# enordber/pepr

Measured on AMD Instinct MI355X. Metric: M site-lnL/sec (WAG+G4 full-tree likelihood evaluations x alignment patterns); the gene-trees/sec half of BASELINE.json's metric is search.gene_trees_per_sec, higher is better.
Workload: dtype f64

## Files before the change

### pepr_amd/csrc/kernels.hip

```cpp
#include "kernels.h"
#include <hip/hip_ext.h>

#include <algorithm>
#include <cstdlib>

namespace pml {

#define TWO_P256 1.15792089237316195423570985008687907853269984665640564039457584007913129639936e77
#define TWO_M256 8.63616855509444462538635186280017219262570580443837358382049248904e-78
#define LOG_2_256 177.445678223345993274051579105116

__device__ __forceinline__ double mfma4(double a, double b, double c) {
#ifdef ABL_NO_MFMA
    return __builtin_fma(a, b, c);
#endif
    return __builtin_amdgcn_mfma_f64_4x4x4f64(a, b, c, 0, 0, 0);
}

__device__ __forceinline__ unsigned code_mask(unsigned code) {
    return code < 20u ? (1u << code) : (code == 20u ? 0xCu : (code == 21u ? 0x60u : 0xFFFFFu));
}

template <int CTRL>
__device__ __forceinline__ double quad_swap(double v) {
// ... 334 lines not shown
typedef double dvec2 __attribute__((ext_vector_type(2)));
typedef int ivec2 __attribute__((ext_vector_type(2)));
typedef unsigned uvec4 __attribute__((ext_vector_type(4)));
struct Operand {
    dvec2 v[5];
};

typedef const __attribute__((address_space(1))) char *gcptr;
typedef __attribute__((address_space(1))) char *gptr;
#define GLOBAL_AS __attribute__((address_space(1)))

__device__ __forceinline__ void load_clv(Operand &o, gcptr base, unsigned lane_off, size_t rowbytes, int c) {
#ifdef ABL_NO_CLV
    { for (int kk = 0; kk < 5; ++kk) o.v[kk] = (dvec2){0.05 + 1e-12 * lane_off, 0.05}; return; }
#endif
#pragma unroll
    for (int kk = 0; kk < 5; ++kk)
        o.v[kk] = __builtin_nontemporal_load(reinterpret_cast<const GLOBAL_AS dvec2 *>(base + (size_t)(c * NS + kk * 4) * rowbytes + lane_off));
}
__device__ __forceinline__ void load_tip(Operand &o, const unsigned char *__restrict__ T, unsigned codes, int q) {
    const unsigned char *t0 = T + (codes & 0xFFu) * NS + q, *t1 = T + (codes >> 8) * NS + q;
#pragma unroll
    for (int kk = 0; kk < 5; ++kk) o.v[kk] = (dvec2){(double)t0[kk * 4], (double)t1[kk * 4]};
}

__device__ __forceinline__ void contract(double (&acc)[5][2], const double *__restrict__ frag_c, const Operand &o) {
#ifdef ABL_NO_LDS
#define FRAG_RD(x) (0.05 + 1.0e-4 * (double)(&(x) - frag_c))
#else
#define FRAG_RD(x) (x)
#endif
    double a[2][5];
#pragma unroll
    for (int st = 0; st < 5; ++st) { acc[st][0] = 0.0; acc[st][1] = 0.0; a[0][st] = FRAG_RD(frag_c[(st * 5) * 16]); }
#pragma unroll
    for (int kk = 0; kk < 5; ++kk) {
        if (kk + 1 < 5) {
#pragma unroll
            for (int st = 0; st < 5; ++st) a[(kk + 1) & 1][st] = FRAG_RD(frag_c[(st * 5 + kk + 1) * 16]);
        }
#pragma unroll
        for (int st = 0; st < 5; ++st) {
            acc[st][0] = mfma4(a[kk & 1][st], o.v[kk].x, acc[st][0]);
            acc[st][1] = mfma4(a[kk & 1][st], o.v[kk].y, acc[st][1]);
        }
        __builtin_amdgcn_sched_barrier(0);
    }
}

template <typename F>
__device__ __forceinline__ void contract_stream(const double *__restrict__ frag_c, const Operand &o, F &&consume) {
    double a[2][5];
#pragma unroll
    for (int kk = 0; kk < 5; ++kk) a[0][kk] = FRAG_RD(frag_c[kk * 16]);
#pragma unroll
    for (int st = 0; st < 5; ++st) {
        if (st + 1 < 5) {
#pragma unroll
            for (int kk = 0; kk < 5; ++kk) a[(st + 1) & 1][kk] = FRAG_RD(frag_c[((st + 1) * 5 + kk) * 16]);
        }
        double acc0 = 0.0, acc1 = 0.0;
#pragma unroll
        for (int kk = 0; kk < 5; ++kk) {
            acc0 = mfma4(a[st & 1][kk], o.v[kk].x, acc0);
            acc1 = mfma4(a[st & 1][kk], o.v[kk].y, acc1);
        }
        consume(st, acc0, acc1);
        __builtin_amdgcn_sched_barrier(0);
    }
}

struct Rows5 { dvec2 a, b; double c; };
__device__ __forceinline__ Rows5 load_rows(const double *tab, unsigned code, int c, int q) {
#ifdef ABL_NO_ROWS
    { Rows5 r1; r1.a = (dvec2){0.9, 0.9}; r1.b = (dvec2){0.9, 0.9}; r1.c = 0.9 + 1e-9 * code; return r1; }
#endif
    gcptr p = (gcptr)tab + (size_t)((c * NCODES + code) * 4 + q) * (TIPTAB_KK * 8);
    Rows5 r;
    r.a = *reinterpret_cast<const GLOBAL_AS dvec2 *>(p);
    r.b = *reinterpret_cast<const GLOBAL_AS dvec2 *>(p + 16);
    r.c = *reinterpret_cast<const GLOBAL_AS double *>(p + 32);
    return r;
}
__device__ __forceinline__ void load_cherry(Operand &o, const OpSide &sd, unsigned ca, unsigned cb, int c, int q) {
    const Rows5 a0 = load_rows(sd.t0, ca & 0xFFu, c, q), a1 = load_rows(sd.t0, ca >> 8, c, q);
    const Rows5 b0 = load_rows(sd.t1, cb & 0xFFu, c, q), b1 = load_rows(sd.t1, cb >> 8, c, q);
    o.v[0] = (dvec2){a0.a.x * b0.a.x, a1.a.x * b1.a.x};
    o.v[1] = (dvec2){a0.a.y * b0.a.y, a1.a.y * b1.a.y};
    o.v[2] = (dvec2){a0.b.x * b0.b.x, a1.b.x * b1.b.x};
    o.v[3] = (dvec2){a0.b.y * b0.b.y, a1.b.y * b1.b.y};
    o.v[4] = (dvec2){a0.c * b0.c, a1.c * b1.c};
}
template <bool EARLY = true>
__device__ __forceinline__ void load_pitch(Operand &o, const OpSide &sd, const double *__restrict__ f_inner,
                                           unsigned ca, unsigned cb, unsigned cc, int c, int q) {
    Operand w;
    load_cherry(w, sd, ca, cb, c, q);
    Rows5 r0, r1;
    if (EARLY) { r0 = load_rows(sd.t2, cc & 0xFFu, c, q); r1 = load_rows(sd.t2, cc >> 8, c, q); }
    double v[5][2];
    contract(v, f_inner + c * 25 * 16, w);
    if (!EARLY) { r0 = load_rows(sd.t2, cc & 0xFFu, c, q); r1 = load_rows(sd.t2, cc >> 8, c, q); }
    o.v[0] = (dvec2){v[0][0] * r0.a.x, v[0][1] * r1.a.x};
    o.v[1] = (dvec2){v[1][0] * r0.a.y, v[1][1] * r1.a.y};
    o.v[2] = (dvec2){v[2][0] * r0.b.x, v[2][1] * r1.b.x};
    o.v[3] = (dvec2){v[3][0] * r0.b.y, v[3][1] * r1.b.y};
    o.v[4] = (dvec2){v[4][0] * r0.c, v[4][1] * r1.c};
}

template <bool CHAIN, bool FUSE>
__device__ __forceinline__ void chunk_op(const NvOp &op, const double *__restrict__ sP, const unsigned char *__restrict__ sT,
                                         int p, int lane, Operand (&X)[4], ivec2 &xsc) {
    const int q = lane >> 4;
    constexpr size_t rowbytes = (size_t)TILE_PAT * 8;
    const size_t tabrow = (size_t)op.mpad * 8;
    const unsigned lane_off = (unsigned)(p >> 7) * (unsigned)(CLV_ROWS * rowbytes) + (unsigned)((size_t)q * rowbytes) + (unsigned)(p & (TILE_PAT - 1)) * 8u;
    const int lk = op.flags & 3, rk = (op.flags >> 2) & 3;
    const bool nt_store = (op.flags & OPF_NT_STORE) != 0;
    const int mode = op.mode;
    const bool chL = CHAIN && (op.flags & OPF_CHAIN_L) != 0, chR = CHAIN && (op.flags & OPF_CHAIN_R) != 0;
    const bool fusedN = FUSE && (op.flags & OPF_FUSED_NEWTON) != 0;
    const bool keep = !(CHAIN && (op.flags & OPF_NO_STORE) != 0) && !fusedN;
    OpSide sdl = op.l, sdr = op.r;
    const int *l_scl = op.l_scl, *r_scl = op.r_scl; int *out_scl = op.out_scl; double *outp = op.out;
#define PML_PIN(x) asm volatile("" : "+s"(x))
    PML_PIN(sdl.p0); PML_PIN(sdl.p1); PML_PIN(sdl.p2); PML_PIN(sdl.t0); PML_PIN(sdl.t1); PML_PIN(sdl.t2); PML_PIN(sdl.f);
    PML_PIN(sdr.p0); PML_PIN(sdr.p1); PML_PIN(sdr.p2); PML_PIN(sdr.t0); PML_PIN(sdr.t1); PML_PIN(sdr.t2); PML_PIN(sdr.f);
    PML_PIN(l_scl); PML_PIN(r_scl); PML_PIN(out_scl); PML_PIN(outp);
    gcptr Lp = (gcptr)sdl.p0, Rp = (gcptr)sdr.p0;
    gptr O = (gptr)outp;
    const __amdgpu_buffer_rsrc_t orsrc = __builtin_amdgcn_make_buffer_rsrc((void *)outp, 0, 0x7FFFFFFF, 0x00020000);
    const double *fL = sP + (q * 4 + (lane & 3));
    const double *fR = fL + PFRAG;
    unsigned mx0 = 0u, mx1 = 0u;
    double site0 = 0.0, site1 = 0.0;
    unsigned cl = 0, cl2 = 0, cl3 = 0, cr = 0, cr2 = 0, cr3 = 0;
    const double *fLi = fL + 2 * PFRAG;
    const bool both_pitch = lk == SK_PITCH && rk == SK_PITCH;
    const double *fRg = sdr.f + (q * 4 + (lane & 3));
#ifdef ABL_NO_CODES
#define CODE_LD(ptr) ((((unsigned)p * 5u + 1u + (unsigned)(size_t)(ptr)) % 20u) | ((((unsigned)p * 3u + 2u) % 20u) << 8))
#else
#define CODE_LD(ptr) (*reinterpret_cast<const GLOBAL_AS unsigned short *>(ptr))
#endif
    if (lk != SK_CLV) cl = CODE_LD(Lp + p);
    if (lk >= SK_CHERRY) cl2 = CODE_LD((gcptr)sdl.p1 + p);
    if (lk == SK_PITCH) cl3 = CODE_LD((gcptr)sdl.p2 + p);
    if (rk != SK_CLV) cr = CODE_LD(Rp + p);
    if (rk >= SK_CHERRY) cr2 = CODE_LD((gcptr)sdr.p1 + p);
    if (rk == SK_PITCH) cr3 = CODE_LD((gcptr)sdr.p2 + p);

    const bool lookL = mode < MODE_EVALUATE && lk == SK_TIP && !__any((cl & 0xFFu) >= 20u || (cl >> 8) >= 20u);
    const bool lookR = mode < MODE_EVALUATE && rk == SK_TIP && !__any((cr & 0xFFu) >= 20u || (cr >> 8) >= 20u);
    const double *tL0 = sP + ((cl & 0xFFu) >> 2) * 16 + (cl & 3u) * 4 + q, *tL1 = sP + ((cl >> 8) >> 2) * 16 + ((cl >> 8) & 3u) * 4 + q;
    const double *tR0 = sP + PFRAG + ((cr & 0xFFu) >> 2) * 16 + (cr & 3u) * 4 + q, *tR1 = sP + PFRAG + ((cr >> 8) >> 2) * 16 + ((cr >> 8) & 3u) * 4 + q;
    Operand curL, curR;
    if (lk == SK_TIP && !lookL) load_tip(curL, sT, cl, q);
    else if (lk == SK_CLV && !chL) load_clv(curL, Lp, lane_off, rowbytes, 0);
    if (rk == SK_TIP && !lookR) load_tip(curR, sT, cr, q);
    else if (rk == SK_CLV && !chR) load_clv(curR, Rp, lane_off, rowbytes, 0);
    constexpr bool DIRECT_IN = CHAIN && !FUSE;
    constexpr int CAT_UNROLL = CHAIN ? NCAT : 1;
#pragma unroll CAT_UNROLL
    for (int c = 0; c < NCAT; ++c) {
        if (FUSE) { if (chL) curL = X[c]; if (chR) curR = X[c]; }
        if (lk == SK_CHERRY) load_cherry(curL, sdl, cl, cl2, c, q);
        else if (lk == SK_PITCH) load_pitch<!FUSE>(curL, sdl, fLi, cl, cl2, cl3, c, q);
        if (rk == SK_CHERRY) load_cherry(curR, sdr, cr, cr2, c, q);
        else if (rk == SK_PITCH) { if (both_pitch) load_pitch<!FUSE>(curR, sdr, fRg, cr, cr2, cr3, c, q); else load_pitch<!FUSE>(curR, sdr, fLi, cr, cr2, cr3, c, q); }
        if (mode >= MODE_EVALUATE) {
            if (DIRECT_IN && chL) contract_stream(fR + c * 25 * 16, curR, [&](int st, double y0, double y1) { site0 += X[c].v[st].x * y0; site1 += X[c].v[st].y * y1; });
            else if (DIRECT_IN && chR) contract_stream(fR + c * 25 * 16, X[c], [&](int st, double y0, double y1) { site0 += curL.v[st].x * y0; site1 += curL.v[st].y * y1; });
            else contract_stream(fR + c * 25 * 16, curR, [&](int st, double y0, double y1) {
                site0 += curL.v[st].x * y0; site1 += curL.v[st].y * y1;
            });
            if (mode == MODE_EVALUATE_CAT) {
                double a0 = site0, a1 = site1;
                a0 += __shfl_xor(a0, 16); a0 += __shfl_xor(a0, 32);
                a1 += __shfl_xor(a1, 16); a1 += __shfl_xor(a1, 32);
                if (q == 0) *reinterpret_cast<GLOBAL_AS dvec2 *>(O + (size_t)c * tabrow + 8 * p) = (dvec2){a0, a1};
                site0 = 0.0; site1 = 0.0;
            }
        } else {
            double aL[5][2];
            if (lookL) {
#pragma unroll
                for (int st = 0; st < 5; ++st) { aL[st][0] = tL0[c * 400 + st * 80]; aL[st][1] = tL1[c * 400 + st * 80]; }
            } else if (DIRECT_IN && chL) contract(aL, fL + c * 25 * 16, X[c]);
            else contract(aL, fL + c * 25 * 16, curL);
            auto emit = [&](int st, double y0, double y1) {
                const double o0 = aL[st][0] * y0, o1 = aL[st][1] * y1;
                mx0 = max(mx0, (unsigned)__double2hiint(o0)); mx1 = max(mx1, (unsigned)__double2hiint(o1));
                if (CHAIN) X[c].v[st] = (dvec2){o0, o1};
                if (!keep) return;
#ifdef ABL_NO_STORE
                return;
#endif
                const uvec4 bits = __builtin_bit_cast(uvec4, ((dvec2){o0, o1}));
                const int soff = (c * NS + st * 4) * (int)rowbytes;
                if (nt_store) __builtin_amdgcn_raw_buffer_store_b128(bits, orsrc, lane_off, soff, 2);
                else __builtin_amdgcn_raw_buffer_store_b128(bits, orsrc, lane_off, soff, 0);
            };
            if (lookR) {
#pragma unroll
                for (int st = 0; st < 5; ++st) emit(st, tR0[c * 400 + st * 80], tR1[c * 400 + st * 80]);
            } else contract_stream(fR + c * 25 * 16, curR, emit);
        }
        if (c + 1 < NCAT) {
            if (lk == SK_CLV && !chL) load_clv(curL, Lp, lane_off, rowbytes, c + 1);
            if (rk == SK_CLV && !chR) load_clv(curR, Rp, lane_off, rowbytes, c + 1);
        }
    }

    ivec2 sc = {0, 0};
    if (q == 0) {
        if (lk == SK_CLV) { if (chL) sc += xsc; else sc += *reinterpret_cast<const GLOBAL_AS ivec2 *>((gcptr)l_scl + 4 * p); }
        if (rk == SK_CLV) { if (chR) sc += xsc; else sc += *reinterpret_cast<const GLOBAL_AS ivec2 *>((gcptr)r_scl + 4 * p); }
    }
    if (mode == MODE_NEWVIEW) {
        mx0 = max(mx0, (unsigned)__shfl_xor((int)mx0, 16)); mx0 = max(mx0, (unsigned)__shfl_xor((int)mx0, 32));
        mx1 = max(mx1, (unsigned)__shfl_xor((int)mx1, 16)); mx1 = max(mx1, (unsigned)__shfl_xor((int)mx1, 32));
        constexpr unsigned HI_TWO_M256 = (1023u - 256u) << 20;
        const bool n0 = mx0 < HI_TWO_M256, n1 = mx1 < HI_TWO_M256;
        if (__any(n0 || n1)) {
            if (CHAIN) {
                const double f0 = n0 ? TWO_P256 : 1.0, f1 = n1 ? TWO_P256 : 1.0;
#pragma unroll
                for (int c = 0; c < NCAT; ++c)
#pragma unroll
                    for (int k = 0; k < 5; ++k) { X[c].v[k].x *= f0; X[c].v[k].y *= f1; }
            }
            if (keep && (n0 || n1)) {
#pragma unroll 1
                for (int r = 0; r < NCAT * 5; ++r) {
                    GLOBAL_AS dvec2 *ptr = reinterpret_cast<GLOBAL_AS dvec2 *>(O + (size_t)((r / 5) * NS + (r % 5) * 4) * rowbytes + lane_off);
                    dvec2 v = *ptr;
                    if (n0) v.x *= TWO_P256;
                    if (n1) v.y *= TWO_P256;
                    *ptr = v;
                }
            }
        }
        if (q == 0) { sc.x += n0 ? 1 : 0; sc.y += n1 ? 1 : 0; if (keep) *reinterpret_cast<GLOBAL_AS ivec2 *>((gptr)out_scl + 4 * p) = sc; }
        if (CHAIN) xsc = sc;
    } else if (mode == MODE_SUMTABLE || mode == MODE_EVALUATE_CAT) {
        if (fusedN) xsc = sc;
        else if (q == 0) *reinterpret_cast<GLOBAL_AS ivec2 *>((gptr)out_scl + 4 * p) = sc;
    } else {
        site0 += __shfl_xor(site0, 16); site0 += __shfl_xor(site0, 32);
        site1 += __shfl_xor(site1, 16); site1 += __shfl_xor(site1, 32);
        if (q == 0) {
            const double l0 = log(site0 * 0.25) - sc.x * LOG_2_256;
            const double l1 = log(site1 * 0.25) - sc.y * LOG_2_256;
            *reinterpret_cast<GLOBAL_AS dvec2 *>(O + 8 * p) = (dvec2){l0, l1};
        }
    }
}

constexpr int PAT_PER_WG = 4 * PAT_PER_WAVE;
constexpr int TIPTAB = NCODES * NS;

#ifndef PML_CHAIN_WAVES
#define PML_CHAIN_WAVES 2
#endif
__device__ __forceinline__ void dma_chunk(const double *set, double *lds_set, int k, int lane) {
    const GLOBAL_AS char *src = (const GLOBAL_AS char *)set + k * 4096 + lane * 16;
    __attribute__((address_space(3))) char *dst = (__attribute__((address_space(3))) char *)lds_set + k * 4096;
    if (k < 3) {
        __builtin_amdgcn_global_load_lds((const GLOBAL_AS void *)src, (__attribute__((address_space(3))) void *)dst, 16, 0, 0);
        __builtin_amdgcn_global_load_lds((const GLOBAL_AS void *)src, (__attribute__((address_space(3))) void *)dst, 16, 1024, 0);
        __builtin_amdgcn_global_load_lds((const GLOBAL_AS void *)src, (__attribute__((address_space(3))) void *)dst, 16, 2048, 0);
        __builtin_amdgcn_global_load_lds((const GLOBAL_AS void *)src, (__attribute__((address_space(3))) void *)dst, 16, 3072, 0);
    } else if (lane < 32) __builtin_amdgcn_global_load_lds((const GLOBAL_AS void *)src, (__attribute__((address_space(3))) void *)dst, 16, 0, 0);
}
__device__ __forceinline__ void stage_frags_dma3(const NvOp &op, double *dst, int lane, int wave) {
    const int wv = __builtin_amdgcn_readfirstlane(wave);
    const double *pl = op.pl, *pr = op.pr;
    const int lk = op.flags & 3, rk = (op.flags >> 2) & 3;
    const double *inner = (lk == SK_PITCH) ? op.l.f : (rk == SK_PITCH) ? op.r.f : nullptr;
    dma_chunk(pl ? pl : pr, dst, wv, lane);
    dma_chunk(pr ? pr : pl, dst + PFRAG, (wv + 1) & 3, lane);
    if (inner != nullptr) dma_chunk(inner, dst + 2 * PFRAG, (wv + 2) & 3, lane);
}

struct FusedShared {
    double exl[NCAT * NS][2];
    double red[3];
    double fb[3][PAT_PER_WAVE * 4];
    double ss[PAT_PER_WAVE * 4];
    double bc[4];
};
static_assert(sizeof(FusedShared) <= PFRAG * sizeof(double), "fused Newton scratch fits one fragment region");
__device__ __forceinline__ void newton_fused(const NvOp &op, double *scratch, const Operand (&X)[4], const ivec2 xsc,
                                             bool active, int blk, NewtonCtl *ctl, long long timeout_ticks) {
    const NewtonReq &r = *reinterpret_cast<const NewtonReq *>(op.aux);
    FusedShared &sh = *reinterpret_cast<FusedShared *>(scratch);
    const int tid = threadIdx.x, lane = tid & 63, wave = tid >> 6, q = lane >> 4, pl = wave * PAT_PER_WAVE + 2 * (lane & 15);
    const int mpad = r.mpad, S = newton_split(mpad);
    const ModelDev *__restrict__ md = r.md;
    u64 *gran = reinterpret_cast<u64 *>(r.sync);
    __syncthreads();
    if (q == 0) { sh.ss[pl] = active ? (double)xsc.x : 0.0; sh.ss[pl + 1] = active ? (double)xsc.y : 0.0; }
    if (tid == 0) sh.bc[3] = 0.0;
    double sw = 0.0;
    if (wave < 2) { const int pf = blk * (PAT_PER_WAVE * 4) + wave * 64 + lane; if (pf < mpad) sw = r.weight[pf]; }
    int nevals = 0;
    auto eval_at = [&](double t, double &L, double &d1, double &d2) -> bool {
        if (tid < NCAT * NS) {
            const double lr = md->eval[tid % NS] * r.rates[tid / NS];
            sh.exl[tid][0] = exp(lr * t); sh.exl[tid][1] = lr;
        }
        __syncthreads();
        double fa = 0.0, fa1 = 0.0, fa2 = 0.0, fb = 0.0, fb1 = 0.0, fb2 = 0.0;
#pragma unroll
        for (int c = 0; c < NCAT; ++c)
#pragma unroll
            for (int st = 0; st < 5; ++st) {
                const int row = c * NS + 4 * st + q;
                const double e = sh.exl[row][0], lr = sh.exl[row][1];
                newton_term(X[c].v[st].x, e, lr, fa, fa1, fa2);
                newton_term(X[c].v[st].y, e, lr, fb, fb1, fb2);
            }
        fa += __shfl_xor(fa, 16); fa += __shfl_xor(fa, 32); fa1 += __shfl_xor(fa1, 16); fa1 += __shfl_xor(fa1, 32); fa2 += __shfl_xor(fa2, 16); fa2 += __shfl_xor(fa2, 32);
        fb += __shfl_xor(fb, 16); fb += __shfl_xor(fb, 32); fb1 += __shfl_xor(fb1, 16); fb1 += __shfl_xor(fb1, 32); fb2 += __shfl_xor(fb2, 16); fb2 += __shfl_xor(fb2, 32);
        if (q == 0) {
            sh.fb[0][pl] = fa; sh.fb[1][pl] = fa1; sh.fb[2][pl] = fa2;
            sh.fb[0][pl + 1] = fb; sh.fb[1][pl + 1] = fb1; sh.fb[2][pl + 1] = fb2;
        }
        __syncthreads();
        double tot[3] = {0.0, 0.0, 0.0};
        if (wave < 2) {
            double a0 = 0.0, a1 = 0.0, a2 = 0.0;
            if (sw != 0.0) {
                const int j = wave * 64 + lane;
                newton_finish(sh.fb[0][j], sh.fb[1][j], sh.fb[2][j], sw, sh.ss[j], a0, a1, a2);
            }
            tot[0] = wave_sum(a0); tot[1] = wave_sum(a1); tot[2] = wave_sum(a2);
            if (wave == 0 && lane == 0) { sh.red[0] = tot[0]; sh.red[1] = tot[1]; sh.red[2] = tot[2]; }
        }
        __syncthreads();
        if (wave == 1) {
#pragma unroll
            for (int i = 0; i < 3; ++i) tot[i] = sh.red[i] + __shfl(tot[i], 0);
            bool bad = false;
            if (S > 1) bad = newton_exchange(gran, S, blk, nevals, r.tag_base, tot, ctl, timeout_ticks);
            if (lane == 0) { sh.bc[0] = tot[0]; sh.bc[1] = tot[1]; sh.bc[2] = tot[2]; if (bad) sh.bc[3] = 1.0; }
        }
        __syncthreads();
        ++nevals;
        L = uni(sh.bc[0]); d1 = uni(sh.bc[1]); d2 = uni(sh.bc[2]);
        return sh.bc[3] == 0.0;
    };
    double t, L, d1, d2;
    const bool ok = newton_drive(r.t0, r.max_iter, r.tol, eval_at, t, L, d1, d2);
    if (tid == 64 && blk == 0) {
        atomicAdd(&ctl->n_requests, 1ull); atomicAdd(&ctl->n_evals, (unsigned long long)nevals);
        if (!ok) { t = r.t0; L = __builtin_nan(""); }
        r.out[0] = t; r.out[1] = L; r.out[2] = d1; r.out[3] = d2;
        if (r.t_dev0) { *r.t_dev0 = t; *r.t_dev1 = t; }
    }
}

#ifdef PML_OPTIME
__device__ unsigned long long g_optime[256][2];
}
extern "C" void pml_abl_optime(unsigned long long *out, int reset) {
    (void)hipDeviceSynchronize();
    (void)hipMemcpyFromSymbol(out, HIP_SYMBOL(pml::g_optime), sizeof(unsigned long long) * 512);
    if (reset) { static unsigned long long z[512]; (void)hipMemcpyToSymbol(HIP_SYMBOL(pml::g_optime), z, sizeof z); }
}
namespace pml {
#endif
template <bool CHAIN, bool DBUF, bool FUSE>
__global__ __launch_bounds__(256, CHAIN ? PML_CHAIN_WAVES : 4) void k_oplist(
        const NvOp *__restrict__ ops, const GeneRun *__restrict__ runs, int nruns, int blocks_per_gene, int any_pitch,
        NewtonCtl *ctl, long long timeout_ticks) {
    static_assert(CHAIN || !DBUF, "LDS-DMA staging exists for the chained kernels only");
    static_assert(!FUSE || (CHAIN && DBUF), "the fused-Newton kernel is the scoring kernel plus the Newton code");
#ifdef PML_OPTIME
    const long long t_life0 = clock64();
#endif
    constexpr int PARITY_STRIDE = 3 * PFRAG;
    Operand X[4]; ivec2 xsc = {0, 0};
#pragma unroll
    for (int c = 0; c < 4; ++c)
#pragma unroll
        for (int k = 0; k < 5; ++k) X[c].v[k] = (dvec2){0.0, 0.0};
    extern __shared__ double sP[];
    const int nfrag_regions = DBUF ? 6 : 2 + (any_pitch ? 1 : 0);
    unsigned char *sT = reinterpret_cast<unsigned char *>(sP + nfrag_regions * PFRAG);
    const int tid = threadIdx.x, lane = tid & 63, wave = tid >> 6;
    const bool one_part = blocks_per_gene < 0;
    if (one_part) blocks_per_gene = -blocks_per_gene;
    const int xcd = one_part ? 0 : (blockIdx.x & 7);
    int slot = one_part ? (int)blockIdx.x : (int)(blockIdx.x >> 3);
    const bool ticketed = FUSE && ctl != nullptr;
    if (ticketed) {
        __shared__ int s_slot;
        if (tid == 0) s_slot = __hip_atomic_fetch_add(&ctl->oticket[xcd], 1, __ATOMIC_RELAXED, __HIP_MEMORY_SCOPE_AGENT);
        __syncthreads();
        slot = s_slot;
    }
    auto leave = [&]() {
        if (!ticketed) return;
        __syncthreads();
        if (tid == 0) {
            const int d = __hip_atomic_fetch_add(&ctl->odone, 1, __ATOMIC_RELAXED, __HIP_MEMORY_SCOPE_AGENT);
            if (d == (int)gridDim.x - 1) {
#pragma unroll
                for (int k = 0; k < 8; ++k) __hip_atomic_store(&ctl->oticket[k], 0, __ATOMIC_RELAXED, __HIP_MEMORY_SCOPE_AGENT);
                __hip_atomic_store(&ctl->odone, 0, __ATOMIC_RELAXED, __HIP_MEMORY_SCOPE_AGENT);
            }
        }
    };
    const int gi = one_part ? slot / blocks_per_gene : xcd + 8 * (slot / blocks_per_gene), blk = slot % blocks_per_gene;
    if (gi >= nruns) { leave(); return; }
    const GeneRun run = runs[gi];
    if (run.op_begin >= run.op_end) { leave(); return; }
    const int mpad = ops[run.op_begin].mpad;
    if (blk * PAT_PER_WG >= mpad) { leave(); return; }
    const int p = (blk * 4 + wave) * PAT_PER_WAVE + 2 * (lane & 15);
    const bool active = (blk * 4 + wave) * PAT_PER_WAVE < mpad;

#ifdef PML_OPTIME
    const long long t_start1 = clock64();
#endif
    for (int i = tid; i < TIPTAB; i += 256) sT[i] = (unsigned char)((code_mask(i / NS) >> (i % NS)) & 1u);
    if (DBUF) stage_frags_dma3(ops[run.op_begin], sP, lane, wave);
    __syncthreads();
#ifdef PML_OPTIME
    const long long t_start2 = clock64();
    long long t_newton = 0, t_bar = 0, t_ops = 0;
#endif
    for (int oi = run.op_begin; oi < run.op_end; ++oi) {
        const NvOp &op = ops[oi];
        const double *buf = sP;
        if (DBUF) {
            const int par = (oi - run.op_begin) & 1;
            buf = sP + par * PARITY_STRIDE;
            if (oi + 1 < run.op_end) stage_frags_dma3(ops[oi + 1], sP + (par ^ 1) * PARITY_STRIDE, lane, wave);
        } else {
            if (oi > run.op_begin) __syncthreads();
            const double2 *gl = reinterpret_cast<const double2 *>(op.pl);
            const double2 *gr = reinterpret_cast<const double2 *>(op.pr);
            double2 *s2 = reinterpret_cast<double2 *>(sP);
            for (int i = tid; i < PFRAG / 2; i += 256) {
                if (op.mode < MODE_EVALUATE && op.pl) s2[i] = gl[i];
                if (op.pr) s2[PFRAG / 2 + i] = gr[i];
            }
            if (any_pitch) {
                const int lk = op.flags & 3, rk = (op.flags >> 2) & 3;
                const double2 *il = reinterpret_cast<const double2 *>(op.l.f), *ir = reinterpret_cast<const double2 *>(op.r.f);
                for (int i = tid; i < PFRAG / 2; i += 256) {
                    if (lk == SK_PITCH) s2[PFRAG + i] = il[i];
                    else if (rk == SK_PITCH) s2[PFRAG + i] = ir[i];
                }
            }
            __syncthreads();
        }
#ifdef PML_OPTIME
        const long long t_op0 = clock64();
#endif
#ifndef ABL_NO_OP
        if (active) chunk_op<CHAIN, FUSE>(op, buf, sT, p, lane, X, xsc);
#endif
#ifdef PML_OPTIME
        if (lane == 0 && active) {
            const int k = (op.flags & 15) | ((op.mode & 3) << 4) | ((op.flags & (OPF_CHAIN_L | OPF_CHAIN_R)) ? 64 : 0) | ((op.flags & OPF_NO_STORE) ? 128 : 0);
            atomicAdd(&g_optime[k][0], (unsigned long long)(clock64() - t_op0)); atomicAdd(&g_optime[k][1], 1ull);
        }
        t_ops += clock64() - t_op0;
        const long long t_n0 = clock64();
#endif
        if (FUSE && (op.flags & OPF_FUSED_NEWTON) != 0) {
            if (__hip_atomic_load(&ctl->abort, __ATOMIC_RELAXED, __HIP_MEMORY_SCOPE_AGENT) != 0) {
                const NewtonReq &r = *reinterpret_cast<const NewtonReq *>(op.aux);
                if (tid == 0 && blk == 0) { r.out[0] = r.t0; r.out[1] = __builtin_nan(""); r.out[2] = 0.0; r.out[3] = 0.0; }
            } else newton_fused(op, const_cast<double *>(buf), X, xsc, active, blk, ctl, timeout_ticks);
        }
#ifdef PML_OPTIME
        const long long t_b0 = clock64(); t_newton += t_b0 - t_n0;
#endif
#ifndef ABL_NO_BARRIER
        if (DBUF) __syncthreads();
#endif
#ifdef PML_OPTIME
        t_bar += clock64() - t_b0;
#endif
    }
#ifdef PML_OPTIME
    if (lane == 0 && active) {
        const int b = FUSE ? 230 : 238;
        const long long t_end = clock64();
        atomicAdd(&g_optime[b][0], (unsigned long long)(t_end - t_life0)); atomicAdd(&g_optime[b][1], 1ull);
        atomicAdd(&g_optime[b + 1][0], (unsigned long long)(t_start1 - t_life0)); atomicAdd(&g_optime[b + 2][0], (unsigned long long)(t_start2 - t_start1));
        atomicAdd(&g_optime[b + 3][0], (unsigned long long)t_ops); atomicAdd(&g_optime[b + 4][0], (unsigned long long)t_newton); atomicAdd(&g_optime[b + 5][0], (unsigned long long)t_bar);
    }
#endif
    leave();
}

constexpr auto k_oplist_plain = k_oplist<false, false, false>;
constexpr auto k_oplist_chain1 = k_oplist<true, false, false>;
constexpr auto k_oplist_score = k_oplist<true, true, false>;
constexpr auto k_oplist_newton = k_oplist<true, true, true>;

template <int N, int WAVES>
__device__ __forceinline__ void block_sum(double (&v)[N], double (*red)[WAVES]) {
    const int lane = threadIdx.x & 63, wave = threadIdx.x >> 6;
#pragma unroll
    for (int i = 0; i < N; ++i) { const double s = wave_sum(v[i]); if (lane == 0) red[i][wave] = s; }
    __syncthreads();
#pragma unroll
    for (int i = 0; i < N; ++i) {
        double s = red[i][0];
#pragma unroll
        for (int w = 1; w < WAVES; ++w) s += red[i][w];
        v[i] = s;
    }
    __syncthreads();
}

__global__ __launch_bounds__(256) void k_reduce(const ReduceReq *__restrict__ reqs) {
    __shared__ double red[1][4];
    const ReduceReq r = reqs[blockIdx.x];
    double acc[1] = {0.0};
    for (int p = threadIdx.x; p < r.mpad; p += 256) {
        const double w = r.weight[p];
        if (w != 0.0) acc[0] += w * r.patlnl[p];
    }
    block_sum<1, 4>(acc, red);
    if (threadIdx.x == 0) *r.out = acc[0];
}

constexpr int NEWTON_THREADS = 512;
constexpr int NEWTON_WAVES = NEWTON_THREADS / 64;
constexpr int NEWTON_SLICE = NEWTON_WAVES * 16;
constexpr int NEWTON_ROWS = CLV_ROWS / 4;
static_assert(NEWTON_SLICE == NEWTON_SLICE_PAT, "kernels.h newton_split / newton_slice describe this kernel's slices");

struct NewtonShared {
    double exl[NCAT * NS][2];
    double red[3][NEWTON_WAVES];
    double fb[3][NEWTON_SLICE];
    double xs[2][NEWTON_ROWS][64];
    double part[3][NEWTON_MAX_SPLIT];
    double bc[4];
    int ticket;
};

template <bool REG, int ROLE, bool SEQ>
__device__ __forceinline__ void newton_body(const NewtonReq &r, NewtonShared &sh, NewtonCtl *ctl,
                                            int S, int wg, int slice, long long timeout_ticks) {
    constexpr bool SVC = ROLE != 0;
    const int tid = threadIdx.x, lane = tid & 63, wave = tid >> 6;
    const int mpad = r.mpad;
    const ModelDev *__restrict__ md = r.md;
    u64 *gran = reinterpret_cast<u64 *>(r.sync);
    int nevals = 0;
    double xr[NEWTON_ROWS]; const int sub = tid & 3;
    double sw = 0.0, ss = 0.0;
    auto row_of = [&](int i) { return (i / 5) * NS + 4 * (i % 5) + sub; };
    auto load_slice = [&](int s) {
        const int p_begin = s * slice, p_end = min(mpad, p_begin + slice);
        const int p = p_begin + (tid >> 2), pc = min(p, p_end - 1);
        const double *col = r.sumtab + clv_index(sub, pc);
        if (SVC) {
#pragma unroll 4
            for (int i = 0; i < NEWTON_ROWS; ++i) sh.xs[ROLE - 1][i][lane] = col[(size_t)((i / 5) * NS + 4 * (i % 5)) * TILE_PAT];
            const int pf = p_begin + 64 * (ROLE - 1) + lane;
            sw = 0.0; ss = 0.0;
            if (pf < p_end) { sw = r.weight[pf]; ss = (double)r.scl[pf]; }
        } else {
#pragma unroll
            for (int i = 0; i < NEWTON_ROWS; ++i) xr[i] = col[(size_t)((i / 5) * NS + 4 * (i % 5)) * TILE_PAT];
        }
    };
    if (REG && !SEQ) load_slice(wg);
    auto fill_exl = [&](double t) {
        if (lane < NCAT * NS / 2) {
            const int k = (ROLE - 1) * (NCAT * NS / 2) + lane;
            const double lr = md->eval[k % NS] * r.rates[k / NS];
// ... 207 lines not shown
    __shared__ double red1[1][4];
    block_sum<1, 4>(cnt, red1);
    if (tid == 0) *r.out = (r.nboot > 0) ? cnt[0] / (double)r.nboot : 0.0;
}

__global__ __launch_bounds__(256) void k_g20(const G20Req *__restrict__ reqs) {
    __shared__ double red[1][4];
    __shared__ double w[G20_RATES];
    const G20Req &r = reqs[blockIdx.x];
    if (threadIdx.x < G20_RATES) w[threadIdx.x] = r.w[threadIdx.x];
    __syncthreads();
    const size_t M = (size_t)r.mpad;
    double acc[1] = {0.0};
    for (int p = threadIdx.x; p < r.mpad; p += 256) {
        const double wt = r.weight[p];
        double l = 0.0;
        if (wt != 0.0) {
            int m = r.cnt[p];
#pragma unroll
            for (int j = 1; j < G20_RATES / 4; ++j) m = min(m, r.cnt[(size_t)j * M + p]);
            double sum = 0.0;
#pragma unroll
            for (int j = 0; j < G20_RATES / 4; ++j) {
                const int d = r.cnt[(size_t)j * M + p] - m;
                const double f = ldexp(1.0, -256 * d);
#pragma unroll
                for (int c = 0; c < 4; ++c) sum += w[4 * j + c] * r.table[(size_t)(4 * j + c) * M + p] * f;
            }
            l = log(sum) - m * LOG_2_256;
            acc[0] += wt * l;
        }
        if (r.patlnl) r.patlnl[p] = l;
    }
    block_sum<1, 4>(acc, red);
    if (threadIdx.x == 0) *r.out = acc[0];
}

void launch_g20(const G20Req *reqs, int n, hipStream_t s) {
    if (n <= 0) return;
    hipLaunchKernelGGL(k_g20, dim3((unsigned)n), dim3(256), 0, s, reqs);
}
void launch_sh(const ShReq *reqs, int n, hipStream_t s) {
    if (n <= 0) return;
    hipLaunchKernelGGL(k_sh, dim3((unsigned)n), dim3(256), 0, s, reqs);
}
void launch_gather(const GatherSeg *segs, int nsegs, int max_npat, hipStream_t s) {
    if (nsegs <= 0 || max_npat <= 0) return;
    hipLaunchKernelGGL(k_gather, dim3((unsigned)nsegs, (unsigned)((max_npat + 255) / 256)), dim3(256), 0, s, segs);
}
void launch_pmat(const ModelDev *model, const PmatReq *reqs, double *frags, int n, hipStream_t s, bool per_request, hipEvent_t start, hipEvent_t stop) {
    if (n <= 0) return;
    const int per_block = PMAT_THREADS / 64;
    const int blocks = std::min((n + per_block - 1) / per_block, 512);
    if (per_request) hipExtLaunchKernelGGL(k_pmat<true>, dim3(blocks), dim3(PMAT_THREADS), 0, s, start, stop, 0, model, reqs, frags, n);
    else hipExtLaunchKernelGGL(k_pmat<false>, dim3(blocks), dim3(PMAT_THREADS), 0, s, start, stop, 0, model, reqs, frags, n);
}
void launch_eigfrags(const ModelDev *model, double *frags2, hipStream_t s) {
    hipLaunchKernelGGL(k_eigfrags, dim3(1), dim3(256), 0, s, model, frags2);
}
void launch_eigfrags_n(const ModelDev *models, double *frags2, int n, hipStream_t s) {
    if (n > 0) hipLaunchKernelGGL(k_eigfrags, dim3((unsigned)n), dim3(256), 0, s, models, frags2);
}
void launch_model_build(const ModelReq *reqs, int n, hipStream_t s, hipEvent_t start, hipEvent_t stop) {
    if (n > 0) hipExtLaunchKernelGGL(k_model, dim3((unsigned)n), dim3(MODEL_THREADS), 0, s, start, stop, 0, reqs);
}
static long long newton_timeout_ticks();
static void launch_oplist_one(const NvOp *ops, const GeneRun *runs, int nruns, int bpg, bool one_part, bool any_pitch, bool chained, hipStream_t s, NewtonCtl *ctl,
                              hipEvent_t start = nullptr, hipEvent_t stop = nullptr);
void launch_oplist(const NvOp *ops, const GeneRun *runs, int nruns, int max_mpad, bool any_pitch, bool chained, hipStream_t s, NewtonCtl *ctl,
                   hipEvent_t start, hipEvent_t stop) {
    if (nruns <= 0) return;
    const int bpg = (max_mpad + PAT_PER_WG - 1) / PAT_PER_WG;
    if (!ctl) { launch_oplist_one(ops, runs, nruns, bpg, false, any_pitch, chained, s, nullptr, start, stop); return; }
    launch_oplist_one(ops, runs, nruns, bpg, bpg > 32, any_pitch, true, s, ctl);
}
static void launch_oplist_one(const NvOp *ops, const GeneRun *runs, int nruns, int bpg_in, bool one_part, bool any_pitch, bool chained, hipStream_t s, NewtonCtl *ctl,
                              hipEvent_t start, hipEvent_t stop) {
    const long long to = newton_timeout_ticks();
    const int bpg = one_part ? -bpg_in : bpg_in;
    const dim3 grid((unsigned)(one_part ? nruns * bpg_in : ((nruns + 7) / 8) * 8 * bpg_in)), block(256);
    const int ap = any_pitch ? 1 : 0;
    const size_t lds_single = (size_t)(2 + ap) * PFRAG * sizeof(double) + 512;
    const size_t lds_double = (size_t)6 * PFRAG * sizeof(double) + 512;
    if (!chained) {
        hipExtLaunchKernelGGL(k_oplist_plain, grid, block, lds_single, s, start, stop, 0, ops, runs, nruns, bpg, ap, ctl, to);
        return;
    }
    static const hipError_t big = [&] {
        const hipError_t a = hipFuncSetAttribute(reinterpret_cast<const void *>(k_oplist_score), hipFuncAttributeMaxDynamicSharedMemorySize, (int)lds_double);
        const hipError_t b = hipFuncSetAttribute(reinterpret_cast<const void *>(k_oplist_newton), hipFuncAttributeMaxDynamicSharedMemorySize, (int)lds_double);
        return a != hipSuccess ? a : b;
    }();
    static const bool want_chain1 = std::getenv("PML_CHAIN_VARIANT") && std::atoi(std::getenv("PML_CHAIN_VARIANT")) == 9;
    if (ctl) hipExtLaunchKernelGGL(k_oplist_newton, grid, block, lds_double, s, start, stop, 0, ops, runs, nruns, bpg, ap, ctl, to);
    else if (want_chain1 || big != hipSuccess) hipExtLaunchKernelGGL(k_oplist_chain1, grid, block, lds_single, s, start, stop, 0, ops, runs, nruns, bpg, ap, ctl, to);
    else hipExtLaunchKernelGGL(k_oplist_score, grid, block, lds_double, s, start, stop, 0, ops, runs, nruns, bpg, ap, ctl, to);
}
void launch_reduce(const ReduceReq *reqs, int n, hipStream_t s, hipEvent_t start, hipEvent_t stop) {
    if (n <= 0) return;
    hipExtLaunchKernelGGL(k_reduce, dim3(n), dim3(256), 0, s, start, stop, 0, reqs);
}
static long long newton_timeout_ticks() {
    static const long long v = [] { const char *e = std::getenv("PML_NEWTON_TIMEOUT_US"); return e ? std::atoll(e) * 100LL : 2000000LL * 100LL; }();
    return v;
}
void launch_newton(const ModelDev *model, const NewtonReq *reqs, const int *tickets, int nreg, int nstream, NewtonCtl *ctl, hipStream_t s) {
    const long long to = newton_timeout_ticks();
    if (nreg > 0) hipLaunchKernelGGL((k_newton<true, false>), dim3((unsigned)nreg), dim3(NEWTON_THREADS), 0, s, model, reqs, tickets, ctl, to);
    if (nstream > 0) hipLaunchKernelGGL((k_newton<false, false>), dim3((unsigned)nstream), dim3(NEWTON_THREADS), 0, s, model, reqs, tickets + nreg, ctl, to);
}
void launch_newton_seq(const ModelDev *model, const NewtonReq *reqs, const int *req_list, int nreg, int nstream, NewtonCtl *ctl, hipStream_t s) {
    if (nreg > 0) hipLaunchKernelGGL((k_newton<true, true>), dim3((unsigned)nreg), dim3(NEWTON_THREADS), 0, s, model, reqs, req_list, ctl, 0LL);
    if (nstream > 0) hipLaunchKernelGGL((k_newton<false, true>), dim3((unsigned)nstream), dim3(NEWTON_THREADS), 0, s, model, reqs, req_list + nreg, ctl, 0LL);
}

}
```

Measured before the change: 175.8.

## Add 8-wave scoring kernel staging fragments and tip tables in LDS

Adds a 512-thread variant of the chained scoring kernel in which each workgroup covers twice as many patterns. The eight waves split the DMA staging of operator fragments, and they also stage the cherry/pitch tip-row tables into LDS. Cherry and pitch loads then read those rows from LDS instead of global memory. The variant is meant to spread fixed per-op staging over more patterns and cut repeated global tip-table loads. In exchange it needs a larger LDS footprint, which may lower occupancy, and the wide path is used only when there are at least two blocks per gene and no Newton control.

```diff
diff --git a/pepr_amd/csrc/kernels.hip b/pepr_amd/csrc/kernels.hip
--- a/pepr_amd/csrc/kernels.hip
+++ b/pepr_amd/csrc/kernels.hip
@@ -440,20 +440,35 @@
     r.c = *reinterpret_cast<const GLOBAL_AS double *>(p + 32);
     return r;
 }
-__device__ __forceinline__ void load_cherry(Operand &o, const OpSide &sd, unsigned ca, unsigned cb, int c, int q) {
-    const Rows5 a0 = load_rows(sd.t0, ca & 0xFFu, c, q), a1 = load_rows(sd.t0, ca >> 8, c, q);
-    const Rows5 b0 = load_rows(sd.t1, cb & 0xFFu, c, q), b1 = load_rows(sd.t1, cb >> 8, c, q);
+__device__ __forceinline__ Rows5 load_rows_lds(const double *tab, unsigned code, int c, int q) {
+#ifdef ABL_NO_ROWS
+    { Rows5 r1; r1.a = (dvec2){0.9, 0.9}; r1.b = (dvec2){0.9, 0.9}; r1.c = 0.9 + 1e-9 * code; return r1; }
+#endif
+    typedef const __attribute__((address_space(3))) char *lcptr;
+    lcptr p = (lcptr)tab + ((c * NCODES + code) * 4 + q) * (TIPTAB_KK * 8);
+    Rows5 r;
+    r.a = *reinterpret_cast<const __attribute__((address_space(3))) dvec2 *>(p);
+    r.b = *reinterpret_cast<const __attribute__((address_space(3))) dvec2 *>(p + 16);
+    r.c = *reinterpret_cast<const __attribute__((address_space(3))) double *>(p + 32);
+    return r;
+}
+template <bool LDS = false>
+__device__ __forceinline__ void load_cherry(Operand &o, const OpSide &sd, const double *sTab, unsigned ca, unsigned cb, int c, int q) {
+    const Rows5 a0 = LDS ? load_rows_lds(sTab, ca & 0xFFu, c, q) : load_rows(sd.t0, ca & 0xFFu, c, q);
+    const Rows5 a1 = LDS ? load_rows_lds(sTab, ca >> 8, c, q) : load_rows(sd.t0, ca >> 8, c, q);
+    const Rows5 b0 = LDS ? load_rows_lds(sTab + TIPTAB_DOUBLES, cb & 0xFFu, c, q) : load_rows(sd.t1, cb & 0xFFu, c, q);
+    const Rows5 b1 = LDS ? load_rows_lds(sTab + TIPTAB_DOUBLES, cb >> 8, c, q) : load_rows(sd.t1, cb >> 8, c, q);
     o.v[0] = (dvec2){a0.a.x * b0.a.x, a1.a.x * b1.a.x};
     o.v[1] = (dvec2){a0.a.y * b0.a.y, a1.a.y * b1.a.y};
     o.v[2] = (dvec2){a0.b.x * b0.b.x, a1.b.x * b1.b.x};
     o.v[3] = (dvec2){a0.b.y * b0.b.y, a1.b.y * b1.b.y};
     o.v[4] = (dvec2){a0.c * b0.c, a1.c * b1.c};
 }
-template <bool EARLY = true>
-__device__ __forceinline__ void load_pitch(Operand &o, const OpSide &sd, const double *__restrict__ f_inner,
+template <bool EARLY = true, bool LDS = false>
+__device__ __forceinline__ void load_pitch(Operand &o, const OpSide &sd, const double *__restrict__ f_inner, const double *sTab,
                                            unsigned ca, unsigned cb, unsigned cc, int c, int q) {
     Operand w;
-    load_cherry(w, sd, ca, cb, c, q);
+    load_cherry<LDS>(w, sd, sTab, ca, cb, c, q);
     Rows5 r0, r1;
     if (EARLY) { r0 = load_rows(sd.t2, cc & 0xFFu, c, q); r1 = load_rows(sd.t2, cc >> 8, c, q); }
     double v[5][2];
@@ -466,7 +481,7 @@
     o.v[4] = (dvec2){v[4][0] * r0.c, v[4][1] * r1.c};
 }
 
-template <bool CHAIN, bool FUSE>
+template <bool CHAIN, bool FUSE, bool TIPLDS = false>
 __device__ __forceinline__ void chunk_op(const NvOp &op, const double *__restrict__ sP, const unsigned char *__restrict__ sT,
                                          int p, int lane, Operand (&X)[4], ivec2 &xsc) {
     const int q = lane >> 4;
@@ -495,6 +510,8 @@
     unsigned cl = 0, cl2 = 0, cl3 = 0, cr = 0, cr2 = 0, cr3 = 0;
     const double *fLi = fL + 2 * PFRAG;
     const bool both_pitch = lk == SK_PITCH && rk == SK_PITCH;
+    const double *sTab = sP + 3 * PFRAG;
+    const bool ldsR = TIPLDS && lk < SK_CHERRY;
     const double *fRg = sdr.f + (q * 4 + (lane & 3));
 #ifdef ABL_NO_CODES
 #define CODE_LD(ptr) ((((unsigned)p * 5u + 1u + (unsigned)(size_t)(ptr)) % 20u) | ((((unsigned)p * 3u + 2u) % 20u) << 8))
@@ -522,10 +539,14 @@
 #pragma unroll CAT_UNROLL
     for (int c = 0; c < NCAT; ++c) {
         if (FUSE) { if (chL) curL = X[c]; if (chR) curR = X[c]; }
-        if (lk == SK_CHERRY) load_cherry(curL, sdl, cl, cl2, c, q);
-        else if (lk == SK_PITCH) load_pitch<!FUSE>(curL, sdl, fLi, cl, cl2, cl3, c, q);
-        if (rk == SK_CHERRY) load_cherry(curR, sdr, cr, cr2, c, q);
-        else if (rk == SK_PITCH) { if (both_pitch) load_pitch<!FUSE>(curR, sdr, fRg, cr, cr2, cr3, c, q); else load_pitch<!FUSE>(curR, sdr, fLi, cr, cr2, cr3, c, q); }
+        if (lk == SK_CHERRY) load_cherry<TIPLDS>(curL, sdl, sTab, cl, cl2, c, q);
+        else if (lk == SK_PITCH) load_pitch<!FUSE, TIPLDS>(curL, sdl, fLi, sTab, cl, cl2, cl3, c, q);
+        if (rk == SK_CHERRY) { if (ldsR) load_cherry<true>(curR, sdr, sTab, cr, cr2, c, q); else load_cherry(curR, sdr, sTab, cr, cr2, c, q); }
+        else if (rk == SK_PITCH) {
+            if (both_pitch) load_pitch<!FUSE>(curR, sdr, fRg, sTab, cr, cr2, cr3, c, q);
+            else if (ldsR) load_pitch<!FUSE, true>(curR, sdr, fLi, sTab, cr, cr2, cr3, c, q);
+            else load_pitch<!FUSE>(curR, sdr, fLi, sTab, cr, cr2, cr3, c, q);
+        }
         if (mode >= MODE_EVALUATE) {
             if (DIRECT_IN && chL) contract_stream(fR + c * 25 * 16, curR, [&](int st, double y0, double y1) { site0 += X[c].v[st].x * y0; site1 += X[c].v[st].y * y1; });
             else if (DIRECT_IN && chR) contract_stream(fR + c * 25 * 16, X[c], [&](int st, double y0, double y1) { site0 += curL.v[st].x * y0; site1 += curL.v[st].y * y1; });
@@ -639,6 +660,42 @@
     dma_chunk(pl ? pl : pr, dst, wv, lane);
     dma_chunk(pr ? pr : pl, dst + PFRAG, (wv + 1) & 3, lane);
     if (inner != nullptr) dma_chunk(inner, dst + 2 * PFRAG, (wv + 2) & 3, lane);
+}
+
+__device__ __forceinline__ void dma_rows4(const double *src, double *lds, int row, int lane) {
+    const GLOBAL_AS char *s = (const GLOBAL_AS char *)src + row * 1024 + lane * 16;
+    __attribute__((address_space(3))) char *d = (__attribute__((address_space(3))) char *)lds + row * 1024;
+    __builtin_amdgcn_global_load_lds((const GLOBAL_AS void *)s, (__attribute__((address_space(3))) void *)d, 16, 0, 0);
+    __builtin_amdgcn_global_load_lds((const GLOBAL_AS void *)s, (__attribute__((address_space(3))) void *)d, 16, 1024, 0);
+    __builtin_amdgcn_global_load_lds((const GLOBAL_AS void *)s, (__attribute__((address_space(3))) void *)d, 16, 2048, 0);
+    __builtin_amdgcn_global_load_lds((const GLOBAL_AS void *)s, (__attribute__((address_space(3))) void *)d, 16, 3072, 0);
+}
+__device__ __forceinline__ void dma_row(const double *src, double *lds, int row, int lane, int nlanes) {
+    const GLOBAL_AS char *s = (const GLOBAL_AS char *)src + row * 1024 + lane * 16;
+    __attribute__((address_space(3))) char *d = (__attribute__((address_space(3))) char *)lds + row * 1024;
+    if (lane < nlanes) __builtin_amdgcn_global_load_lds((const GLOBAL_AS void *)s, (__attribute__((address_space(3))) void *)d, 16, 0, 0);
+}
+static_assert(PFRAG * 8 == 12 * 1024 + 32 * 16 && TIPTAB_DOUBLES * 8 == 17 * 1024 + 16 * 16, "rows of a fragment set and of a tip table");
+__device__ __forceinline__ void stage_frags_wide(const NvOp &op, double *dst, int lane, int wave) {
+    const int wv = __builtin_amdgcn_readfirstlane(wave);
+    const double *pl = op.pl, *pr = op.pr;
+    const int lk = op.flags & 3, rk = (op.flags >> 2) & 3;
+    const double *inner = (lk == SK_PITCH) ? op.l.f : (rk == SK_PITCH) ? op.r.f : nullptr;
+    const double *L = pl ? pl : pr, *R = pr ? pr : pl;
+    if (wv < 3) dma_rows4(L, dst, 4 * wv, lane);
+    else if (wv < 6) dma_rows4(R, dst + PFRAG, 4 * (wv - 3), lane);
+    else dma_row(wv == 6 ? L : R, wv == 6 ? dst : dst + PFRAG, 12, lane, 32);
+    if (inner != nullptr) {
+        if (wv >= 5) dma_rows4(inner, dst + 2 * PFRAG, 4 * (wv - 5), lane);
+        else if (wv == 4) dma_row(inner, dst + 2 * PFRAG, 12, lane, 32);
+    }
+    if (lk >= SK_CHERRY || rk >= SK_CHERRY) {
+        const double *ta = lk >= SK_CHERRY ? op.l.t0 : op.r.t0, *tb = lk >= SK_CHERRY ? op.l.t1 : op.r.t1;
+        double *da = dst + 3 * PFRAG, *db = da + TIPTAB_DOUBLES;
+        if (wv < 4) dma_rows4(ta, da, 4 * wv, lane); else dma_rows4(tb, db, 4 * (wv - 4), lane);
+        if (wv < 2) dma_row(ta, da, 16 + wv, lane, wv == 0 ? 64 : 16);
+        else if (wv < 4) dma_row(tb, db, 14 + wv, lane, wv == 2 ? 64 : 16);
+    }
 }
 
 struct FusedShared {
@@ -729,24 +786,27 @@
 }
 namespace pml {
 #endif
-template <bool CHAIN, bool DBUF, bool FUSE>
-__global__ __launch_bounds__(256, CHAIN ? PML_CHAIN_WAVES : 4) void k_oplist(
+template <bool CHAIN, bool DBUF, bool FUSE, int WAVES>
+__device__ __forceinline__ void oplist_body(
         const NvOp *__restrict__ ops, const GeneRun *__restrict__ runs, int nruns, int blocks_per_gene, int any_pitch,
         NewtonCtl *ctl, long long timeout_ticks) {
     static_assert(CHAIN || !DBUF, "LDS-DMA staging exists for the chained kernels only");
     static_assert(!FUSE || (CHAIN && DBUF), "the fused-Newton kernel is the scoring kernel plus the Newton code");
+    static_assert(WAVES == 4 || (WAVES == 8 && CHAIN && DBUF && !FUSE), "eight waves: the scoring kernel only");
+    constexpr bool WIDE = WAVES == 8;
+    constexpr int WG_PAT = WAVES * PAT_PER_WAVE;
 #ifdef PML_OPTIME
     const long long t_life0 = clock64();
 #endif
-    constexpr int PARITY_STRIDE = 3 * PFRAG;
+    constexpr int PARITY_STRIDE = 3 * PFRAG + (WIDE ? 2 * TIPTAB_DOUBLES : 0);
     Operand X[4]; ivec2 xsc = {0, 0};
 #pragma unroll
     for (int c = 0; c < 4; ++c)
 #pragma unroll
         for (int k = 0; k < 5; ++k) X[c].v[k] = (dvec2){0.0, 0.0};
     extern __shared__ double sP[];
-    const int nfrag_regions = DBUF ? 6 : 2 + (any_pitch ? 1 : 0);
-    unsigned char *sT = reinterpret_cast<unsigned char *>(sP + nfrag_regions * PFRAG);
+    const int nfrag_doubles = DBUF ? 2 * PARITY_STRIDE : (2 + (any_pitch ? 1 : 0)) * PFRAG;
+    unsigned char *sT = reinterpret_cast<unsigned char *>(sP + nfrag_doubles);
     const int tid = threadIdx.x, lane = tid & 63, wave = tid >> 6;
     const bool one_part = blocks_per_gene < 0;
     if (one_part) blocks_per_gene = -blocks_per_gene;
@@ -776,15 +836,16 @@
     const GeneRun run = runs[gi];
     if (run.op_begin >= run.op_end) { leave(); return; }
     const int mpad = ops[run.op_begin].mpad;
-    if (blk * PAT_PER_WG >= mpad) { leave(); return; }
-    const int p = (blk * 4 + wave) * PAT_PER_WAVE + 2 * (lane & 15);
-    const bool active = (blk * 4 + wave) * PAT_PER_WAVE < mpad;
+    if (blk * WG_PAT >= mpad) { leave(); return; }
+    const int p = (blk * WAVES + wave) * PAT_PER_WAVE + 2 * (lane & 15);
+    const bool active = (blk * WAVES + wave) * PAT_PER_WAVE < mpad;
 
 #ifdef PML_OPTIME
     const long long t_start1 = clock64();
 #endif
-    for (int i = tid; i < TIPTAB; i += 256) sT[i] = (unsigned char)((code_mask(i / NS) >> (i % NS)) & 1u);
-    if (DBUF) stage_frags_dma3(ops[run.op_begin], sP, lane, wave);
+    for (int i = tid; i < TIPTAB; i += 64 * WAVES) sT[i] = (unsigned char)((code_mask(i / NS) >> (i % NS)) & 1u);
+    auto stage = [&](const NvOp &o, double *dst) { if (WIDE) stage_frags_wide(o, dst, lane, wave); else stage_frags_dma3(o, dst, lane, wave); };
+    if (DBUF) stage(ops[run.op_begin], sP);
     __syncthreads();
 #ifdef PML_OPTIME
     const long long t_start2 = clock64();
@@ -796,7 +857,7 @@
         if (DBUF) {
             const int par = (oi - run.op_begin) & 1;
             buf = sP + par * PARITY_STRIDE;
-            if (oi + 1 < run.op_end) stage_frags_dma3(ops[oi + 1], sP + (par ^ 1) * PARITY_STRIDE, lane, wave);
+            if (oi + 1 < run.op_end) stage(ops[oi + 1], sP + (par ^ 1) * PARITY_STRIDE);
         } else {
             if (oi > run.op_begin) __syncthreads();
             const double2 *gl = reinterpret_cast<const double2 *>(op.pl);
@@ -820,7 +881,7 @@
         const long long t_op0 = clock64();
 #endif
 #ifndef ABL_NO_OP
-        if (active) chunk_op<CHAIN, FUSE>(op, buf, sT, p, lane, X, xsc);
+        if (active) chunk_op<CHAIN, FUSE, WIDE>(op, buf, sT, p, lane, X, xsc);
 #endif
 #ifdef PML_OPTIME
         if (lane == 0 && active) {
@@ -856,6 +917,17 @@
     }
 #endif
     leave();
+}
+template <bool CHAIN, bool DBUF, bool FUSE>
+__global__ __launch_bounds__(256, CHAIN ? PML_CHAIN_WAVES : 4) void k_oplist(
+        const NvOp *__restrict__ ops, const GeneRun *__restrict__ runs, int nruns, int blocks_per_gene, int any_pitch,
+        NewtonCtl *ctl, long long timeout_ticks) {
+    oplist_body<CHAIN, DBUF, FUSE, 4>(ops, runs, nruns, blocks_per_gene, any_pitch, ctl, timeout_ticks);
+}
+__global__ __launch_bounds__(512, PML_CHAIN_WAVES) void k_oplist_wide(
+        const NvOp *__restrict__ ops, const GeneRun *__restrict__ runs, int nruns, int blocks_per_gene, int any_pitch,
+        NewtonCtl *ctl, long long timeout_ticks) {
+    oplist_body<true, true, false, 8>(ops, runs, nruns, blocks_per_gene, any_pitch, ctl, timeout_ticks);
 }
 
 constexpr auto k_oplist_plain = k_oplist<false, false, false>;
@@ -1229,6 +1301,7 @@
     const int ap = any_pitch ? 1 : 0;
     const size_t lds_single = (size_t)(2 + ap) * PFRAG * sizeof(double) + 512;
     const size_t lds_double = (size_t)6 * PFRAG * sizeof(double) + 512;
+    const size_t lds_wide = (size_t)2 * (3 * PFRAG + 2 * TIPTAB_DOUBLES) * sizeof(double) + 512;
     if (!chained) {
         hipExtLaunchKernelGGL(k_oplist_plain, grid, block, lds_single, s, start, stop, 0, ops, runs, nruns, bpg, ap, ctl, to);
         return;
@@ -1238,7 +1311,14 @@
         const hipError_t b = hipFuncSetAttribute(reinterpret_cast<const void *>(k_oplist_newton), hipFuncAttributeMaxDynamicSharedMemorySize, (int)lds_double);
         return a != hipSuccess ? a : b;
     }();
-    static const bool want_chain1 = std::getenv("PML_CHAIN_VARIANT") && std::atoi(std::getenv("PML_CHAIN_VARIANT")) == 9;
+    static const int variant = std::getenv("PML_CHAIN_VARIANT") ? std::atoi(std::getenv("PML_CHAIN_VARIANT")) : 0;
+    static const bool want_chain1 = variant == 9;
+    static const hipError_t big_wide = hipFuncSetAttribute(reinterpret_cast<const void *>(k_oplist_wide), hipFuncAttributeMaxDynamicSharedMemorySize, (int)lds_wide);
+    if (!ctl && !one_part && variant == 0 && big_wide == hipSuccess && bpg_in > 1) {
+        const int bpg_wide = (bpg_in + 1) / 2;
+        hipExtLaunchKernelGGL(k_oplist_wide, dim3((unsigned)(((nruns + 7) / 8) * 8 * bpg_wide)), dim3(512), lds_wide, s, start, stop, 0, ops, runs, nruns, bpg_wide, ap, ctl, to);
+        return;
+    }
     if (ctl) hipExtLaunchKernelGGL(k_oplist_newton, grid, block, lds_double, s, start, stop, 0, ops, runs, nruns, bpg, ap, ctl, to);
     else if (want_chain1 || big != hipSuccess) hipExtLaunchKernelGGL(k_oplist_chain1, grid, block, lds_single, s, start, stop, 0, ops, runs, nruns, bpg, ap, ctl, to);
     else hipExtLaunchKernelGGL(k_oplist_score, grid, block, lds_double, s, start, stop, 0, ops, runs, nruns, bpg, ap, ctl, to);
```

Result: faster. 190.6 (median of 6 runs) (+8.4%).
